# prisma-lab/WBC-quadruped-DOB

Hardware: AMD Instinct MI355X
Metric: WBC control-steps/sec (batched DogBot) (higher is better)
Workload: dtype f64; 1 GPU; configs[1]: batch=4096 states/GPU, 4-contact stance, observer off, f64; synthetic quadruped URDF (DogBot URDF absent); batch_per_gpu=4096, parallelism=batch-sharded x1, no data-path collective, writes_M_h_Jc=True

## Files before the change

### wbc_quadruped_dob_amd/csrc/dyn_split.hip.hpp

```cpp
#pragma once
#include <hip/hip_runtime.h>
#include <type_traits>
#include "device_types.hpp"
#include "dyn_sweep.hip.hpp"

namespace wbc {


#define WBC_LAUNDERED_TID(name) unsigned name = threadIdx.x; asm volatile("" : "+v"(name))
#define WBC_ADDR_MACROS                                                                                                   \
  const size_t N = a.N;                                                                                                    \
  const unsigned N32 = (unsigned)N;                                                                                        \
                                                      \
  const int leg = (int)((tx & 63) >> 4);                                                                          \
     \
  const size_t s_raw = EXT ? (size_t)blockIdx.x * SPW + (tx & 15)                                                 \
                           : ((size_t)blockIdx.x * (BLOCK / 64) + (tx >> 6)) * 16 + (tx & 15);           \
  const bool slot_ok = SPW == 16 || (int)(tx & 15) < SPW;                                                                  \
  const bool live = slot_ok && s_raw < N;                                                                                  \
  unsigned s32 = (unsigned)(live ? s_raw : (slot_ok ? N - 1 : (size_t)blockIdx.x * SPW));                                  \
  const unsigned legN = (unsigned)leg * N32;
#define WBC_STATE_MACROS                                                                                                                          \
  constexpr bool SIMG = EXT == 3;                     \
  const T* const si_ = SIMG ? a.simg + (int)(s32 - (unsigned)((size_t)blockIdx.x * SPW)) : nullptr;                                               \
  auto ldq = [&](int comp) __attribute__((always_inline)) -> T { if constexpr (SIMG) return si_[comp * 16]; else return LDU(a.q, comp); };         \
  auto ldv = [&](int comp) __attribute__((always_inline)) -> T { if constexpr (SIMG) return si_[(SIMG_V + comp) * 16]; else return LDU(a.v, comp); }; \
  (void)ldq; (void)ldv;
#define LDQJ(k_) (SIMG ? si_[(7 + jx[k_]) * 16] : LDX(a.q, 7, jxN[k_]))
#define LDVJ(k_) (SIMG ? si_[(SIMG_V + 6 + jx[k_]) * 16] : LDX(a.v, 6, jxN[k_]))
#define CS(i) cst[(i) * 4 + leg]
#define LDU(ptr, comp) (*(const T*)((const char*)((ptr) + (size_t)(comp) * N) + (size_t)(s32 * (unsigned)sizeof(T))))
#define LDV(ptr, comp) (*(const T*)((const char*)(ptr) + (size_t)(((unsigned)(comp) * N32 + s32) * (unsigned)sizeof(T))))
#define LDX(ptr, c0, xN) (*(const T*)((const char*)((ptr) + (size_t)(c0) * N) + (size_t)(((xN) + s32) * (unsigned)sizeof(T))))
#define WBC_ROLE_LIVE ((0 && EXT != 0) || live)
#define STV(ptr, comp, val) do { if (WBC_ROLE_LIVE) *(T*)((char*)(ptr) + (size_t)(((unsigned)(comp) * N32 + s32) * (unsigned)sizeof(T))) = (val); } while (0)
#define STVG(ptr, comp, val) do { if (live) *(T*)((char*)(ptr) + (size_t)(((unsigned)(comp) * N32 + s32) * (unsigned)sizeof(T))) = (val); } while (0)
#define STL(ptr, c0, stride, val) do { if (WBC_ROLE_LIVE) *(T*)((char*)((ptr) + (size_t)(c0) * N) + (size_t)(((unsigned)(stride) * legN + s32) * (unsigned)sizeof(T))) = (val); } while (0)
#define STLX(ptr, c0, stride, xN, val) do { if (WBC_ROLE_LIVE) *(T*)((char*)((ptr) + (size_t)(c0) * N) + (size_t)(((unsigned)(stride) * legN + (xN) + s32) * (unsigned)sizeof(T))) = (val); } while (0)
#define ST4(ptr, c0, v0_, c1, v1_, c2, v2_, c3, v3_) STV(ptr, sel4<int>(leg, c0, c1, c2, c3), sel4<T>(leg, v0_, v1_, v2_, v3_))
#define ST4G(ptr, c0, v0_, c1, v1_, c2, v2_, c3, v3_) STVG(ptr, sel4<int>(leg, c0, c1, c2, c3), sel4<T>(leg, v0_, v1_, v2_, v3_))
#define MAKE_R(R_, qx, qy, qz, qw) do { const T x = qx, y = qy, z = qz, w = qw; \
    R_.a[0] = 1 - 2 * (y * y + z * z); R_.a[1] = 2 * (x * y - z * w);     R_.a[2] = 2 * (x * z + y * w); \
    R_.a[3] = 2 * (x * y + z * w);     R_.a[4] = 1 - 2 * (x * x + z * z); R_.a[5] = 2 * (y * z - x * w); \
    R_.a[6] = 2 * (x * z - y * w);     R_.a[7] = 2 * (y * z + x * w);     R_.a[8] = 1 - 2 * (x * x + y * y); } while (0)

constexpr int WBC_MJ_WAVES = 2;
constexpr int WBC_RS_WAVES = 2;

template <class T>
WBC_DEV void structural_consts_quarter(const DevModel<T>* __restrict__ model, const SweepArgs<T>& a, const int* zidx_s, unsigned tx) {
  const size_t N = a.N;
  const unsigned N32 = (unsigned)N;
  const int leg = (int)((tx >> 4) & 3), part = (int)(tx >> 6);
  const size_t s_raw = (size_t)blockIdx.x * 16 + (tx & 15);
  const bool live = s_raw < N;
  const unsigned s32 = (unsigned)(live ? s_raw : N - 1);
  const T Z = (T)0;
  int jq[3];
  jidx_of_leg(model, a.jpack, leg, jq);
  const int j0 = jq[0], j1 = jq[1], j2 = jq[2];
  if ((N & 1) == 0) {
    struct alignas(2 * sizeof(T)) T2 { T a, b; };
    const unsigned odd = s32 & 1u, s2 = s32 & ~1u;
#define ST2C(ptr, comp, val) do { if (live) *(T2*)((char*)(ptr) + (size_t)(((unsigned)(comp) * N32 + s2) * (unsigned)sizeof(T))) = T2{(val), (val)}; } while (0)
    if (part == 3) {
      for (int e = 2 * leg + (int)odd; e < 64; e += 8) {
        const int zi = zidx_s[e];
        if (zi >= 0) ST2C(a.M, zi, Z);
      }
    } else {
      const int mrow = part;
      const int rb = 54 * leg + 18 * mrow;
      ST2C(a.Jc, rb + (odd ? 1 : 0), ((odd ? 1 : 0) == mrow) ? (T)1 : Z);
      ST2C(a.Jc, rb + (odd ? 3 + mrow : 2), (!odd && mrow == 2) ? (T)1 : Z);
#pragma unroll
      for (int c = 6; c < 18; c += 2) {
        const int col = c + (int)odd - 6;
        if (col != j0 && col != j1 && col != j2) ST2C(a.Jc, rb + c + (int)odd, Z);
      }
    }
#undef ST2C
  } else {
#define ST1C(ptr, comp, val) do { if (live) *(T*)((char*)(ptr) + (size_t)(((unsigned)(comp) * N32 + s32) * (unsigned)sizeof(T))) = (val); } while (0)
    if (part == 3) {
      for (int e = leg; e < 64; e += 4) {
        const int zi = zidx_s[e];
        if (zi >= 0) ST1C(a.M, zi, Z);
      }
    } else {
      const int mrow = part;
      const int rb = 54 * leg + 18 * mrow;
#pragma unroll
      for (int c = 0; c < 3; ++c) ST1C(a.Jc, rb + c, (c == mrow) ? (T)1 : Z);
      ST1C(a.Jc, rb + 3 + mrow, Z);
#pragma unroll
      for (int c = 0; c < 12; ++c)
        if (c != j0 && c != j1 && c != j2) ST1C(a.Jc, rb + 6 + c, Z);
    }
#undef ST1C
  }
}

constexpr int MJ_HAND_WORDS = 46;
struct MjNoHook { WBC_DEV void operator()() const {} };
template <class T, int BLOCK, int EXT, int SPW = 16, int ZEROS = 1, class AfterHand = MjNoHook>
WBC_DEV void mass_jac_body(const DevModel<T>* __restrict__ model, const SweepArgs<T>& a, const T* cst_ext, const int* zidx_ext, T* hand = nullptr,
                           AfterHand after_hand = AfterHand()) {
  static_assert(!EXT || BLOCK == 64 || BLOCK == 128, "one wavefront (128: one of the two role wavefronts of a fused_pair_kernel workgroup, each with its own half of the parking lot)");
  static_assert(SPW == 16 || EXT != 0, "fewer states per workgroup only for roles");
  WBC_LAUNDERED_TID(tx);
  __shared__ __attribute__((aligned(512))) T cst_own[EXT ? 1 : CST_WORDS];
  __shared__ int zidx_own[EXT ? 1 : 64];
  if constexpr (EXT == 0) {
    for (int i = tx; i < CST_WORDS; i += blockDim.x) cst_own[i] = model->cst[i];
    if (tx < 64) zidx_own[tx] = model->zidx[tx];
    __syncthreads();
  }
  const T* cst = EXT ? cst_ext : cst_own;
  const int* zidx_s = EXT ? zidx_ext : zidx_own;
  WBC_ADDR_MACROS
  WBC_STATE_MACROS
  const bool direct = hand == nullptr;

  T qq[4];
#pragma unroll
  for (int c = 0; c < 4; ++c) qq[c] = ldq(3 + c);
  int jx[3];
  unsigned jxN[3];
  jidx_of_leg(model, a.jpack, leg, jx);
#pragma unroll
  for (int k = 0; k < 3; ++k) jxN[k] = (unsigned)jx[k] * N32;
  T ql[3];
#pragma unroll
  for (int k = 0; k < 3; ++k) ql[k] = LDQJ(k);
  if constexpr (EXT == 2) __syncthreads();

  auto write_consts = [&]() __attribute__((always_inline)) {
    const T Z = (T)0;
    for (int e = leg; e < 64; e += 4) {
      const int zi = zidx_s[e];
      if (zi >= 0) STV(a.M, zi, Z);
    }
#pragma unroll
    for (int mrow = 0; mrow < 3; ++mrow) {
#pragma unroll
      for (int c = 0; c < 3; ++c) STL(a.Jc, 18 * mrow + c, 54, (c == mrow) ? (T)1 : Z);
      STL(a.Jc, 18 * mrow + 3 + mrow, 54, Z);
#pragma unroll
      for (int c = 0; c < 12; ++c)
        if (c != jx[0] && c != jx[1] && c != jx[2]) STL(a.Jc, 18 * mrow + 6 + c, 54, Z);
    }
  };
  if constexpr (ZEROS == 1) { if (!a.skip_consts) write_consts(); }
  T qx, qy, qz, qw;
  {
    const T n = rsqrt_sel<SIMG>(qq[0] * qq[0] + qq[1] * qq[1] + qq[2] * qq[2] + qq[3] * qq[3]);
    qx = qq[0] * n; qy = qq[1] * n; qz = qq[2] * n; qw = qq[3] * n;
  }
  __shared__ T park[18][BLOCK];
  const int ln = EXT ? (int)(tx & (unsigned)(BLOCK - 1)) : (int)tx;
  T* const hl = hand ? hand + (int)(tx & 63) : nullptr;
  M3<T> E2;
#pragma unroll
  for (int k = 0; k < 3; ++k) {
    const int o = JOINT_WORDS * k;
    T sn, cs;
    sincos_t(ql[k], &sn, &cs);
#pragma unroll
    for (int e = 0; e < 9; ++e) {
      const T v = CS(o + e) + cs * CS(o + 9 + e) + sn * CS(o + 18 + e);
      if (k < 2) park[9 * k + e][ln] = v; else E2.a[e] = v;
    }
  }
  T cm; V3<T> ch; S3<T> cI;
  V3<T> dft = mk<T>(CS(129), CS(130), CS(131));
  V3<T> jc[3];
  SF<T> Fp[3];
#pragma unroll
  for (int k = 2; k >= 0; --k) {
    const int o = JOINT_WORDS * k;
    const V3<T> r = mk<T>(CS(o + 27), CS(o + 28), CS(o + 29));
    const V3<T> ax = mk<T>(CS(o + 30), CS(o + 31), CS(o + 32));
    const T m = CS(o + 33);
    const V3<T> h = mk<T>(CS(o + 34), CS(o + 35), CS(o + 36));
    S3<T> Io;
    Io.xx = CS(o + 37); Io.xy = CS(o + 38); Io.xz = CS(o + 39); Io.yy = CS(o + 40); Io.yz = CS(o + 41); Io.zz = CS(o + 42);
    M3<T> E;
    if (k == 2) E = E2;
    else {
#pragma unroll
      for (int e = 0; e < 9; ++e) E.a[e] = park[9 * k + e][ln];
    }
    if (k == 2) { cm = m; ch = h; cI = Io; }
    else {
      cm += m; ch = ch + h;
      cI.xx += Io.xx; cI.xy += Io.xy; cI.xz += Io.xz; cI.yy += Io.yy; cI.yz += Io.yz; cI.zz += Io.zz;
    }
    Fp[k].n = mul(cI, ax);
    Fp[k].f = cross(ax, ch);
#pragma unroll
    for (int j = k; j < 3; ++j) {
      const T mkj = dot(ax, Fp[j].n);
      if (direct) {
        int i = 6 + jx[k], jj = 6 + jx[j];
        if (i > jj) { const int t = i; i = jj; jj = t; }
        STV(a.M, i * 18 - i * (i - 1) / 2 + (jj - i), mkj);
      } else hl[(k * 3 - k * (k - 1) / 2 + (j - k)) * 64] = mkj;
    }
    jc[k] = cross(ax, dft);
    dft = r + mul(E, dft);
#pragma unroll
    for (int j = k; j < 3; ++j) { jc[j] = mul(E, jc[j]); Fp[j] = to_parent(E, r, Fp[j]); }
    {
      const V3<T> hr = mul(E, ch);
      const S3<T> Ir = congr(E, cI);
      const V3<T> w = hr + r * (cm * (T)0.5);
      const T sc = 2 * dot(w, r);
      cI.xx = Ir.xx + sc - 2 * w.x * r.x;
      cI.yy = Ir.yy + sc - 2 * w.y * r.y;
      cI.zz = Ir.zz + sc - 2 * w.z * r.z;
      cI.xy = Ir.xy - (w.x * r.y + r.x * w.y);
      cI.xz = Ir.xz - (w.x * r.z + r.x * w.z);
      cI.yz = Ir.yz - (w.y * r.z + r.y * w.z);
      ch = hr + r * cm;
    }
  }
  M3<T> R;
  MAKE_R(R, qx, qy, qz, qw);
  const V3<T> dw = mul(R, dft);
#pragma unroll
  for (int k = 0; k < 3; ++k) {
    const V3<T> Mf = mul(R, Fp[k].f), Mn = mul(R, Fp[k].n);
    const V3<T> jw = mul(R, jc[k]);
    if (direct) {
      const unsigned x = jxN[k];
      STLX(a.M, 6, 0, x, Mf.x);
      STLX(a.M, midx18(1, 1) + 5, 0, x, Mf.y);
      STLX(a.M, midx18(2, 2) + 4, 0, x, Mf.z);
      STLX(a.M, midx18(3, 3) + 3, 0, x, Mn.x);
      STLX(a.M, midx18(4, 4) + 2, 0, x, Mn.y);
      STLX(a.M, midx18(5, 5) + 1, 0, x, Mn.z);
      STLX(a.Jc, 0 * 18 + 6, 54, x, jw.x);
      STLX(a.Jc, 1 * 18 + 6, 54, x, jw.y);
      STLX(a.Jc, 2 * 18 + 6, 54, x, jw.z);
    } else {
      hl[(6 + 0 + k) * 64] = Mf.x; hl[(6 + 3 + k) * 64] = Mf.y; hl[(6 + 6 + k) * 64] = Mf.z;
      hl[(6 + 9 + k) * 64] = Mn.x; hl[(6 + 12 + k) * 64] = Mn.y; hl[(6 + 15 + k) * 64] = Mn.z;
      hl[(24 + 0 + k) * 64] = jw.x; hl[(24 + 3 + k) * 64] = jw.y; hl[(24 + 6 + k) * 64] = jw.z;
    }
  }
  if (direct) {
    STL(a.Jc, 0 * 18 + 4, 54, dw.z);  STL(a.Jc, 0 * 18 + 5, 54, -dw.y);
    STL(a.Jc, 1 * 18 + 3, 54, -dw.z); STL(a.Jc, 1 * 18 + 5, 54, dw.x);
    STL(a.Jc, 2 * 18 + 3, 54, dw.y);  STL(a.Jc, 2 * 18 + 4, 54, -dw.x);
    if (a.pf) {
      STL(a.pf, 0, 3, ldq(0) + dw.x);
      STL(a.pf, 1, 3, ldq(1) + dw.y);
      STL(a.pf, 2, 3, ldq(2) + dw.z);
    }
  } else {
    hl[33 * 64] = dw.x; hl[34 * 64] = dw.y; hl[35 * 64] = dw.z;
    if (!a.skip_mats && a.pf) {
      STL(a.pf, 0, 3, ldq(0) + dw.x);
      STL(a.pf, 1, 3, ldq(1) + dw.y);
      STL(a.pf, 2, 3, ldq(2) + dw.z);
    }
  }
  {
    const T bm = model->base_m;
    const V3<T> bh = mk<T>(model->base_h[0], model->base_h[1], model->base_h[2]);
    const T tm = xrow_sum(cm) + bm;
    const V3<T> th = xrow_sum(ch) + bh;
    S3<T> tI;
    tI.xx = xrow_sum(cI.xx) + model->base_Io[0]; tI.xy = xrow_sum(cI.xy) + model->base_Io[1]; tI.xz = xrow_sum(cI.xz) + model->base_Io[2];
    tI.yy = xrow_sum(cI.yy) + model->base_Io[3]; tI.yz = xrow_sum(cI.yz) + model->base_Io[4]; tI.zz = xrow_sum(cI.zz) + model->base_Io[5];
    const V3<T> hw = mul(R, th);
    const S3<T> Iw = congr(R, tI);
    if (direct) {
      T* M = a.M;
      ST4(M, midx18(0, 0), tm, midx18(1, 1), tm, midx18(2, 2), tm, midx18(0, 4), hw.z);
      ST4(M, midx18(0, 5), -hw.y, midx18(1, 3), -hw.z, midx18(1, 5), hw.x, midx18(2, 3), hw.y);
      ST4(M, midx18(2, 4), -hw.x, midx18(3, 3), Iw.xx, midx18(3, 4), Iw.xy, midx18(3, 5), Iw.xz);
      if (leg < 3) STV(M, sel4<int>(leg, midx18(4, 4), midx18(4, 5), midx18(5, 5), 0), sel4<T>(leg, Iw.yy, Iw.yz, Iw.zz, Iw.zz));
    } else {
      hl[36 * 64] = tm; hl[37 * 64] = hw.x; hl[38 * 64] = hw.y; hl[39 * 64] = hw.z;
      hl[40 * 64] = Iw.xx; hl[41 * 64] = Iw.xy; hl[42 * 64] = Iw.xz; hl[43 * 64] = Iw.yy; hl[44 * 64] = Iw.yz; hl[45 * 64] = Iw.zz;
    }
  }
  if (!direct) {
    after_hand();
    if (!a.skip_mats) {
#pragma unroll
      for (int k = 0; k < 3; ++k) {
#pragma unroll
        for (int j = k; j < 3; ++j) {
          int i = 6 + jx[k], jj = 6 + jx[j];
          if (i > jj) { const int t = i; i = jj; jj = t; }
          STV(a.M, i * 18 - i * (i - 1) / 2 + (jj - i), hl[(k * 3 - k * (k - 1) / 2 + (j - k)) * 64]);
        }
        const unsigned x = jxN[k];
        STLX(a.M, 6, 0, x, hl[(6 + 0 + k) * 64]);
        STLX(a.M, midx18(1, 1) + 5, 0, x, hl[(6 + 3 + k) * 64]);
        STLX(a.M, midx18(2, 2) + 4, 0, x, hl[(6 + 6 + k) * 64]);
        STLX(a.M, midx18(3, 3) + 3, 0, x, hl[(6 + 9 + k) * 64]);
        STLX(a.M, midx18(4, 4) + 2, 0, x, hl[(6 + 12 + k) * 64]);
        STLX(a.M, midx18(5, 5) + 1, 0, x, hl[(6 + 15 + k) * 64]);
        STLX(a.Jc, 0 * 18 + 6, 54, x, hl[(24 + 0 + k) * 64]);
        STLX(a.Jc, 1 * 18 + 6, 54, x, hl[(24 + 3 + k) * 64]);
        STLX(a.Jc, 2 * 18 + 6, 54, x, hl[(24 + 6 + k) * 64]);
      }
      const T dx = hl[33 * 64], dy = hl[34 * 64], dz = hl[35 * 64];
      STL(a.Jc, 0 * 18 + 4, 54, dz);  STL(a.Jc, 0 * 18 + 5, 54, -dy);
      STL(a.Jc, 1 * 18 + 3, 54, -dz); STL(a.Jc, 1 * 18 + 5, 54, dx);
      STL(a.Jc, 2 * 18 + 3, 54, dy);  STL(a.Jc, 2 * 18 + 4, 54, -dx);
      const T tm = hl[36 * 64], hwx = hl[37 * 64], hwy = hl[38 * 64], hwz = hl[39 * 64];
      T* M = a.M;
      ST4(M, midx18(0, 0), tm, midx18(1, 1), tm, midx18(2, 2), tm, midx18(0, 4), hwz);
      ST4(M, midx18(0, 5), -hwy, midx18(1, 3), -hwz, midx18(1, 5), hwx, midx18(2, 3), hwy);
      ST4(M, midx18(2, 4), -hwx, midx18(3, 3), hl[40 * 64], midx18(3, 4), hl[41 * 64], midx18(3, 5), hl[42 * 64]);
      if (leg < 3) STV(M, sel4<int>(leg, midx18(4, 4), midx18(4, 5), midx18(5, 5), 0), sel4<T>(leg, hl[43 * 64], hl[44 * 64], hl[45 * 64], hl[45 * 64]));
    }
  }
  if constexpr (ZEROS == 2) { if (!a.skip_consts) write_consts(); }
}

template <class T, int BLOCK>
__global__ __launch_bounds__(BLOCK, WBC_MJ_WAVES) void mass_jac_kernel(const DevModel<T>* __restrict__ model, SweepArgs<T> a) {
  mass_jac_body<T, BLOCK, 0>(model, a, nullptr, nullptr);
}

struct NoWait { WBC_DEV void operator()() const {} };
template <class T, int MODE, int BLOCK, int EXT, int SPW = 16, class BeforeRefs = NoWait, class AfterGeom = NoWait, class AfterTaup = NoWait>
WBC_DEV void rnea_step_body(const DevModel<T>* __restrict__ model, const DevParams<T> prm, const SweepArgs<T>& a, const T* cst_ext,
                            T* wsl, BeforeRefs before_refs = BeforeRefs(), AfterGeom after_geom = AfterGeom(), T* hres = nullptr, AfterTaup after_taup = AfterTaup()) {
  static_assert(!EXT || BLOCK == 64 || BLOCK == 128, "one wavefront (128: one of the two role wavefronts of a fused_pair_kernel workgroup, each with its own half of the parking lot)");
  WBC_LAUNDERED_TID(tx);
  constexpr bool WH = (MODE & RS_H) != 0, STEP = (MODE & RS_STEP) != 0, OBS = (MODE & RS_OBS) != 0, WPF = (MODE & RS_PF) != 0, FWD_B = (MODE & RS_NOB) == 0;
  constexpr bool OBSW = (MODE & RS_OBSW) != 0;
  static_assert(!OBSW || (EXT != 0 && OBS && !STEP && !WH), "the observer role exists only inside the fused tick");
  constexpr bool NOJC = (MODE & RS_NOJC) != 0;
  static_assert(!NOJC || (EXT != 0 && STEP && !OBS && !WPF), "RS_NOJC: a step role next to a mass_jac role");
  constexpr bool GEOM = (STEP && !NOJC) || OBS || WPF;
  constexpr bool LANE2 = (MODE & RS_LANE2) != 0;
  static_assert(!LANE2 || (EXT != 0 && SPW == 4 && STEP && WH && !OBS), "RS_LANE2: a role of 4-state workgroups that wants h and tau_partial");
  constexpr bool TWO = STEP && WH && !LANE2;
  constexpr bool BASEROWS = WH || OBS;
  constexpr bool EARLY = EXT != 0 && STEP;
  __shared__ __attribute__((aligned(512))) T cst_own[EXT ? 1 : CST_WORDS];
  if constexpr (EXT == 0) {
    for (int i = tx; i < CST_WORDS; i += blockDim.x) cst_own[i] = model->cst[i];
    __syncthreads();
  }
  const T* cst = EXT ? cst_ext : cst_own;
  WBC_ADDR_MACROS
  const bool chainB = LANE2 && (int)(tx & 15) >= SPW && (int)(tx & 15) < 2 * SPW;
  if constexpr (LANE2) {
    if (chainB) { const size_t sb = (size_t)blockIdx.x * SPW + (tx & 15) - SPW; s32 = (unsigned)(sb < N ? sb : N - 1); }
  }
#define WSTV(comp, val) do { if constexpr (EXT != 0) wsl[(comp) * 16 + (int)(tx & 15)] = (val); else STV(a.ws, comp, val); } while (0)
#define WST4(c0, v0_, c1, v1_, c2, v2_, c3, v3_) WSTV(sel4<int>(leg, c0, c1, c2, c3), sel4<T>(leg, v0_, v1_, v2_, v3_))
#define WSTL(c0, stride, val) WSTV((c0) + (stride) * leg, val)

  WBC_STATE_MACROS
  T qq[4], vb[6];
#pragma unroll
  for (int c = 0; c < 4; ++c) qq[c] = ldq(3 + c);
#pragma unroll
  for (int c = 0; c < 6; ++c) vb[c] = ldv(c);
  T qpos[3] = {0, 0, 0};
  if (WPF && a.pf) {
#pragma unroll
    for (int c = 0; c < 3; ++c) qpos[c] = ldq(c);
  }
  int jx[3];
  unsigned jxN[3];
  jidx_of_leg(model, a.jpack, leg, jx);
#pragma unroll
  for (int k = 0; k < 3; ++k) jxN[k] = (unsigned)jx[k] * N32;
  T ql[3], vl[3], al[3] = {0, 0, 0}, ad[6] = {0, 0, 0, 0, 0, 0};
#pragma unroll
  for (int k = 0; k < 3; ++k) { ql[k] = LDQJ(k); vl[k] = LDVJ(k); }
  constexpr bool LATE_REFS = EARLY && !std::is_same<BeforeRefs, NoWait>::value;
  T bw[6] = {0, 0, 0, 0, 0, 0};
  constexpr bool RIMG = (MODE & RS_REFIMG) != 0;
  static_assert(!RIMG || (SIMG && STEP), "RS_REFIMG: a step role of a 4-state rollout workgroup");
  auto load_refs = [&]() __attribute__((always_inline)) {
    before_refs();
    const T* const ri = RIMG ? a.refimg + (si_ - a.simg) : nullptr;
    if (STEP) {
#pragma unroll
      for (int k = 0; k < 3; ++k) al[k] = RIMG ? ri[(6 + 6 + jx[k]) * 16] : LDX(a.vdot_des, 6, jxN[k]);
#pragma unroll
      for (int c = 0; c < 6; ++c) ad[c] = RIMG ? ri[(6 + c) * 16] : LDU(a.vdot_des, c);
    }
    if (STEP && !OBS && FWD_B) {
#pragma unroll
      for (int c = 0; c < 6; ++c) bw[c] = RIMG ? ri[c * 16] : LDU(a.w_des, c);
    }
  };
  if constexpr (!LATE_REFS) load_refs();
  auto lane2_mask = [&]() __attribute__((always_inline)) {
    if constexpr (LANE2) {
#pragma unroll
      for (int c = 0; c < 6; ++c) { vb[c] = chainB ? (T)0 : vb[c]; ad[c] = chainB ? ad[c] : (T)0; }
#pragma unroll
      for (int k = 0; k < 3; ++k) { vl[k] = chainB ? (T)0 : vl[k]; al[k] = chainB ? al[k] : (T)0; }
    }
  };
  if constexpr (!LATE_REFS) lane2_mask();
  if constexpr (EXT == 2) __syncthreads();
  if constexpr (!EARLY) {
    if (STEP && !OBS && FWD_B) {
      WST4(WS_B + 0, bw[0], WS_B + 1, bw[1], WS_B + 2, bw[2], WS_B + 3, bw[3]);
      if (leg < 2) WSTV(WS_B + 4 + leg, leg == 0 ? bw[4] : bw[5]);
    }
  }
  T qx, qy, qz, qw;
  {
    const T n = rsqrt_sel<(SIMG || (0 && EXT == 2))>(qq[0] * qq[0] + qq[1] * qq[1] + qq[2] * qq[2] + qq[3] * qq[3]);
    qx = qq[0] * n; qy = qq[1] * n; qz = qq[2] * n; qw = qq[3] * n;
  }
  T sn3[3] = {0, 0, 0}, cs3[3] = {0, 0, 0};
  constexpr bool KEEP_E = EARLY && SIMG && SPW == 4;
  M3<T> Ekeep[KEEP_E ? 3 : 1];
  if constexpr (EARLY) {
#pragma unroll
    for (int k = 0; k < 3; ++k) sincos_t(ql[k], &sn3[k], &cs3[k]);
    V3<T> d = mk<T>(CS(129), CS(130), CS(131));
#pragma unroll
    for (int k = 2; k >= 0; --k) {
      const int o = JOINT_WORDS * k;
      T s_ = sn3[k], c_ = cs3[k];
      if constexpr (!KEEP_E) asm volatile("" : "+v"(s_), "+v"(c_));
      M3<T> E;
#pragma unroll
      for (int e = 0; e < 9; ++e) E.a[e] = CS(o + e) + c_ * CS(o + 9 + e) + s_ * CS(o + 18 + e);
      if constexpr (KEEP_E) Ekeep[k] = E;
      d = mk<T>(CS(o + 27), CS(o + 28), CS(o + 29)) + mul(E, d);
    }
    M3<T> R0;
    MAKE_R(R0, qx, qy, qz, qw);
    const V3<T> dw0 = mul(R0, d);
    WSTL(WS_D + 0, 3, dw0.x);
    WSTL(WS_D + 1, 3, dw0.y);
    WSTL(WS_D + 2, 3, dw0.z);
    after_geom();
    if constexpr (LATE_REFS) { load_refs(); lane2_mask(); }
    if (STEP && !OBS && FWD_B) {
      WST4(WS_B + 0, bw[0], WS_B + 1, bw[1], WS_B + 2, bw[2], WS_B + 3, bw[3]);
      if (leg < 2) WSTV(WS_B + 4 + leg, leg == 0 ? bw[4] : bw[5]);
    }
    after_geom();
  }
  const T bm = model->base_m;
  const V3<T> bh = mk<T>(model->base_h[0], model->base_h[1], model->base_h[2]);
  S3<T> bI;
  bI.xx = model->base_Io[0]; bI.xy = model->base_Io[1]; bI.xz = model->base_Io[2];
  bI.yy = model->base_Io[3]; bI.yz = model->base_Io[4]; bI.zz = model->base_Io[5];

  constexpr int PW = 15 + (TWO ? 6 : 0) + (OBS ? 18 : 0);
  constexpr int PB = BASEROWS ? (OBS ? 18 : 6) : 1;
  __shared__ T park[2 * PW + PB][BLOCK];
  const int ln = EXT ? (int)(tx & (unsigned)(BLOCK - 1)) : (int)tx;
  constexpr int OFF_A = 15, OFF_O = 15 + (TWO ? 6 : 0);

  V3<T> omp, vp, aAp, aLp, gLp, a2Ap, a2Lp;
  {
    M3<T> R;
    MAKE_R(R, qx, qy, qz, qw);
    const V3<T> om0 = tmul(R, mk<T>(vb[3], vb[4], vb[5]));
    const V3<T> v0 = tmul(R, mk<T>(vb[0], vb[1], vb[2]));
    V3<T> gneg = tmul(R, mk<T>(-model->grav[0], -model->grav[1], -model->grav[2]));
    if constexpr (LANE2) { gneg.x = chainB ? (T)0 : gneg.x; gneg.y = chainB ? (T)0 : gneg.y; gneg.z = chainB ? (T)0 : gneg.z; }
    const V3<T> aL0 = gneg - cross(om0, v0);
    if (BASEROWS) {
      const SF<T> Iv0 = inertia_mul(bm, bh, bI, om0, v0);
      const SF<T> Ia0 = inertia_mul(bm, bh, bI, mk<T>(0, 0, 0), aL0);
      T* pb = &park[2 * PW][ln];
      const V3<T> bwn = Ia0.n + cross(om0, Iv0.n) + cross(v0, Iv0.f), bwf = Ia0.f + cross(om0, Iv0.f);
      pb[0] = bwn.x; pb[BLOCK] = bwn.y; pb[BLOCK * 2] = bwn.z; pb[BLOCK * 3] = bwf.x; pb[BLOCK * 4] = bwf.y; pb[BLOCK * 5] = bwf.z;
      if (OBS) {
        const V3<T> gn = cross(bh, gneg), gf = gneg * bm;
        pb[BLOCK * 6] = Iv0.n.x; pb[BLOCK * 7] = Iv0.n.y; pb[BLOCK * 8] = Iv0.n.z; pb[BLOCK * 9] = Iv0.f.x; pb[BLOCK * 10] = Iv0.f.y; pb[BLOCK * 11] = Iv0.f.z;
        pb[BLOCK * 12] = gn.x; pb[BLOCK * 13] = gn.y; pb[BLOCK * 14] = gn.z; pb[BLOCK * 15] = gf.x; pb[BLOCK * 16] = gf.y; pb[BLOCK * 17] = gf.z;
      }
    }
    omp = om0; vp = v0; aAp = mk<T>(0, 0, 0); aLp = aL0; gLp = gneg;
    a2Ap = tmul(R, mk<T>(ad[3], ad[4], ad[5]));
    a2Lp = tmul(R, mk<T>(ad[0], ad[1], ad[2]));
    if (STEP && !TWO) { aAp = aAp + a2Ap; aLp = aLp + a2Lp; }
  }

  M3<T> E2;
  SF<T> f2, fa2, m2, g2;
  V3<T> om2, vv2;
#pragma unroll
  for (int k = 0; k < 3; ++k) {
    const int o = JOINT_WORDS * k;
    T sn, cs;
    if constexpr (EARLY) { sn = sn3[k]; cs = cs3[k]; }
    else sincos_t(ql[k], &sn, &cs);
    M3<T> E;
    if constexpr (KEEP_E) E = Ekeep[k];
    else {
#pragma unroll
      for (int e = 0; e < 9; ++e) E.a[e] = CS(o + e) + cs * CS(o + 9 + e) + sn * CS(o + 18 + e);
    }
    const V3<T> r = mk<T>(CS(o + 27), CS(o + 28), CS(o + 29));
    const V3<T> ax = mk<T>(CS(o + 30), CS(o + 31), CS(o + 32));
    const T m = CS(o + 33);
    const V3<T> h = mk<T>(CS(o + 34), CS(o + 35), CS(o + 36));
    S3<T> Io;
    Io.xx = CS(o + 37); Io.xy = CS(o + 38); Io.xz = CS(o + 39); Io.yy = CS(o + 40); Io.yz = CS(o + 41); Io.zz = CS(o + 42);
    const T qd = vl[k];
    const V3<T> om = tmul(E, omp) + ax * qd;
    const V3<T> vv = tmul(E, vp + cross(omp, r));
    V3<T> aA = tmul(E, aAp) + cross(om, ax) * qd;
    const V3<T> aL = tmul(E, aLp + cross(aAp, r)) + cross(vv, ax) * qd;
    if (STEP && !TWO) aA = aA + ax * al[k];
    const SF<T> Iv = inertia_mul(m, h, Io, om, vv);
    const SF<T> Ia = inertia_mul(m, h, Io, aA, aL);
    SF<T> fk, fak, gk;
    fk.n = Ia.n + cross(om, Iv.n) + cross(vv, Iv.f);
    fk.f = Ia.f + cross(om, Iv.f);
    if (TWO) {
      const V3<T> a2A = tmul(E, a2Ap) + ax * al[k];
      const V3<T> a2L = tmul(E, a2Lp + cross(a2Ap, r));
      fak = inertia_mul(m, h, Io, a2A, a2L);
      a2Ap = a2A; a2Lp = a2L;
    }
    if (OBS) {
      const V3<T> gL = tmul(E, gLp);
      gk.n = cross(h, gL);
      gk.f = gL * m;
      gLp = gL;
    }
    if (k < 2) {
      T* pk = &park[PW * k][ln];
#pragma unroll
      for (int e = 0; e < 9; ++e) pk[BLOCK * e] = E.a[e];
      pk[BLOCK * 9] = fk.n.x; pk[BLOCK * 10] = fk.n.y; pk[BLOCK * 11] = fk.n.z;
      pk[BLOCK * 12] = fk.f.x; pk[BLOCK * 13] = fk.f.y; pk[BLOCK * 14] = fk.f.z;
      if (TWO) {
        pk[BLOCK * (OFF_A + 0)] = fak.n.x; pk[BLOCK * (OFF_A + 1)] = fak.n.y; pk[BLOCK * (OFF_A + 2)] = fak.n.z;
        pk[BLOCK * (OFF_A + 3)] = fak.f.x; pk[BLOCK * (OFF_A + 4)] = fak.f.y; pk[BLOCK * (OFF_A + 5)] = fak.f.z;
      }
      if (OBS) {
        pk[BLOCK * (OFF_O + 0)] = Iv.n.x; pk[BLOCK * (OFF_O + 1)] = Iv.n.y; pk[BLOCK * (OFF_O + 2)] = Iv.n.z;
        pk[BLOCK * (OFF_O + 3)] = Iv.f.x; pk[BLOCK * (OFF_O + 4)] = Iv.f.y; pk[BLOCK * (OFF_O + 5)] = Iv.f.z;
        pk[BLOCK * (OFF_O + 6)] = gk.n.x; pk[BLOCK * (OFF_O + 7)] = gk.n.y; pk[BLOCK * (OFF_O + 8)] = gk.n.z;
        pk[BLOCK * (OFF_O + 9)] = gk.f.x; pk[BLOCK * (OFF_O + 10)] = gk.f.y; pk[BLOCK * (OFF_O + 11)] = gk.f.z;
        pk[BLOCK * (OFF_O + 12)] = om.x; pk[BLOCK * (OFF_O + 13)] = om.y; pk[BLOCK * (OFF_O + 14)] = om.z;
        pk[BLOCK * (OFF_O + 15)] = vv.x; pk[BLOCK * (OFF_O + 16)] = vv.y; pk[BLOCK * (OFF_O + 17)] = vv.z;
      }
    } else {
      E2 = E; f2 = fk;
      if (TWO) fa2 = fak;
      if (OBS) { m2 = Iv; g2 = gk; om2 = om; vv2 = vv; }
    }
    omp = om; vp = vv; aAp = aA; aLp = aL;
  }

  T p_leg[3], ct_leg[3], g_leg[3], taup[3] = {0, 0, 0};
  const bool h_mem = !(hres != nullptr && a.skip_mats != 0);
  V3<T> dft = mk<T>(CS(129), CS(130), CS(131));
  V3<T> jc[3];
  SF<T> facc, aacc, macc, gacc;
#pragma unroll
  for (int k = 2; k >= 0; --k) {
    const int o = JOINT_WORDS * k;
    const V3<T> r = mk<T>(CS(o + 27), CS(o + 28), CS(o + 29));
    const V3<T> ax = mk<T>(CS(o + 30), CS(o + 31), CS(o + 32));
    M3<T> E;
    SF<T> fk, fak, mk_, gk;
    V3<T> om, vv;
    if (k == 2) {
      E = E2; fk = f2;
      if (TWO) fak = fa2;
      if (OBS) { mk_ = m2; gk = g2; om = om2; vv = vv2; }
    } else {
      const T* pk = &park[PW * k][ln];
#pragma unroll
      for (int e = 0; e < 9; ++e) E.a[e] = pk[BLOCK * e];
      fk.n = mk<T>(pk[BLOCK * 9], pk[BLOCK * 10], pk[BLOCK * 11]) + facc.n;
      fk.f = mk<T>(pk[BLOCK * 12], pk[BLOCK * 13], pk[BLOCK * 14]) + facc.f;
      if (TWO) {
        fak.n = mk<T>(pk[BLOCK * (OFF_A + 0)], pk[BLOCK * (OFF_A + 1)], pk[BLOCK * (OFF_A + 2)]) + aacc.n;
        fak.f = mk<T>(pk[BLOCK * (OFF_A + 3)], pk[BLOCK * (OFF_A + 4)], pk[BLOCK * (OFF_A + 5)]) + aacc.f;
      }
      if (OBS) {
        mk_.n = mk<T>(pk[BLOCK * (OFF_O + 0)], pk[BLOCK * (OFF_O + 1)], pk[BLOCK * (OFF_O + 2)]) + macc.n;
        mk_.f = mk<T>(pk[BLOCK * (OFF_O + 3)], pk[BLOCK * (OFF_O + 4)], pk[BLOCK * (OFF_O + 5)]) + macc.f;
        gk.n = mk<T>(pk[BLOCK * (OFF_O + 6)], pk[BLOCK * (OFF_O + 7)], pk[BLOCK * (OFF_O + 8)]) + gacc.n;
        gk.f = mk<T>(pk[BLOCK * (OFF_O + 9)], pk[BLOCK * (OFF_O + 10)], pk[BLOCK * (OFF_O + 11)]) + gacc.f;
        om = mk<T>(pk[BLOCK * (OFF_O + 12)], pk[BLOCK * (OFF_O + 13)], pk[BLOCK * (OFF_O + 14)]);
        vv = mk<T>(pk[BLOCK * (OFF_O + 15)], pk[BLOCK * (OFF_O + 16)], pk[BLOCK * (OFF_O + 17)]);
      }
    }
    {
      const T hk = dot(ax, fk.n);
      if (WH) {
        unsigned long long jp = a.jpack;
        asm volatile("" : "+s"(jp));
        const unsigned jx_k = ((unsigned)(jp >> (12 * leg)) >> (4 * k)) & 15u;
        const unsigned jxN_k = jx_k * N32;
        if (h_mem) STLX(a.h, 6, 0, jxN_k, hk);
        if (hres) hres[(6 + (int)jx_k) * 16 + (int)(tx & 15)] = hk;
      }
      if (STEP) taup[k] = hk + (TWO ? dot(ax, fak.n) : (T)0);
    }
    if (OBS) {
      p_leg[k] = dot(ax, mk_.n);
      ct_leg[k] = -dot(ax, cross(om, mk_.n) + cross(vv, mk_.f));
      g_leg[k] = dot(ax, gk.n);
    }
    if (GEOM) {
      jc[k] = cross(ax, dft);
      dft = r + mul(E, dft);
#pragma unroll
      for (int j = k; j < 3; ++j) jc[j] = mul(E, jc[j]);
    }
    if (k > 0 || BASEROWS) facc = to_parent(E, r, fk);
    if (TWO && k > 0) aacc = to_parent(E, r, fak);
    if (OBS) { macc = to_parent(E, r, mk_); gacc = to_parent(E, r, gk); }
  }

  M3<T> R;
  MAKE_R(R, qx, qy, qz, qw);
  V3<T> dw = mk<T>(0, 0, 0), jw[3];
  if (GEOM) {
    dw = mul(R, dft);
#pragma unroll
    for (int k = 0; k < 3; ++k) jw[k] = mul(R, jc[k]);
  }
  if (WPF && a.pf) {
    STL(a.pf, 0, 3, qpos[0] + dw.x);
    STL(a.pf, 1, 3, qpos[1] + dw.y);
    STL(a.pf, 2, 3, qpos[2] + dw.z);
  }
  if (STEP) {
    if constexpr (!EARLY) {
      WSTL(WS_D + 0, 3, dw.x);
      WSTL(WS_D + 1, 3, dw.y);
      WSTL(WS_D + 2, 3, dw.z);
    }
    if constexpr (GEOM) {
#pragma unroll
      for (int k = 0; k < 3; ++k) {
        WSTL(WS_JCL + 0 + k, 9, jw[k].x);
        WSTL(WS_JCL + 3 + k, 9, jw[k].y);
        WSTL(WS_JCL + 6 + k, 9, jw[k].z);
      }
    }
  }
  constexpr bool TAUP_FIRST = STEP && !OBS && !OBSW && WH && !std::is_same<AfterTaup, NoWait>::value;
  if constexpr (TAUP_FIRST) {
    if constexpr (LANE2) {
#pragma unroll
      for (int k = 0; k < 3; ++k) taup[k] += dpp_mov<0x12C>(taup[k]);
    }
#pragma unroll
    for (int k = 0; k < 3; ++k) WSTL(WS_TAUP + k, 3, taup[k]);
    after_taup();
  }
  if (WH) {
    const T* pb = &park[2 * PW][ln];
    const V3<T> bfn = xrow_sum(facc.n) + mk<T>(pb[0], pb[BLOCK], pb[BLOCK * 2]);
    const V3<T> bff = xrow_sum(facc.f) + mk<T>(pb[BLOCK * 3], pb[BLOCK * 4], pb[BLOCK * 5]);
    const V3<T> hb_f = mul(R, bff), hb_n = mul(R, bfn);
    if (h_mem) {
      ST4(a.h, 0, hb_f.x, 1, hb_f.y, 2, hb_f.z, 3, hb_n.x);
      if (leg < 2) STV(a.h, 4 + leg, leg == 0 ? hb_n.y : hb_n.z);
    }
    if (hres) {
      hres[sel4<int>(leg, 0, 1, 2, 3) * 16 + (int)(tx & 15)] = sel4<T>(leg, hb_f.x, hb_f.y, hb_f.z, hb_n.x);
      if (leg < 2) hres[(4 + leg) * 16 + (int)(tx & 15)] = leg == 0 ? hb_n.y : hb_n.z;
    }
  }
  T p_b[6], beta_b[6], beta_l[3];
  if (OBS) {
    const T* pb = &park[2 * PW][ln];
    SF<T> mom0, grv0;
    mom0.n = xrow_sum(macc.n) + mk<T>(pb[BLOCK * 6], pb[BLOCK * 7], pb[BLOCK * 8]);
    mom0.f = xrow_sum(macc.f) + mk<T>(pb[BLOCK * 9], pb[BLOCK * 10], pb[BLOCK * 11]);
    grv0.n = xrow_sum(gacc.n) + mk<T>(pb[BLOCK * 12], pb[BLOCK * 13], pb[BLOCK * 14]);
    grv0.f = xrow_sum(gacc.f) + mk<T>(pb[BLOCK * 15], pb[BLOCK * 16], pb[BLOCK * 17]);
    const V3<T> Pl = mul(R, mom0.f), Pa = mul(R, mom0.n);
    const V3<T> gl = mul(R, grv0.f), ga = mul(R, grv0.n);
    const V3<T> cx = cross(mk<T>(vb[0], vb[1], vb[2]), Pl);
    p_b[0] = Pl.x; p_b[1] = Pl.y; p_b[2] = Pl.z; p_b[3] = Pa.x; p_b[4] = Pa.y; p_b[5] = Pa.z;
    beta_b[0] = -gl.x; beta_b[1] = -gl.y; beta_b[2] = -gl.z;
    beta_b[3] = -cx.x - ga.x; beta_b[4] = -cx.y - ga.y; beta_b[5] = -cx.z - ga.z;
#pragma unroll
    for (int k = 0; k < 3; ++k) beta_l[k] = ct_leg[k] - g_leg[k];
    if (a.p) {
      ST4(a.p, 0, p_b[0], 1, p_b[1], 2, p_b[2], 3, p_b[3]);
      if (leg < 2) STV(a.p, 4 + leg, leg == 0 ? p_b[4] : p_b[5]);
#pragma unroll
      for (int k = 0; k < 3; ++k) STLX(a.p, 6, 0, jxN[k], p_leg[k]);
    }
    if (a.beta) {
      ST4(a.beta, 0, beta_b[0], 1, beta_b[1], 2, beta_b[2], 3, beta_b[3]);
      if (leg < 2) STV(a.beta, 4 + leg, leg == 0 ? beta_b[4] : beta_b[5]);
#pragma unroll
      for (int k = 0; k < 3; ++k) STLX(a.beta, 6, 0, jxN[k], beta_l[k]);
    }
  }
  if (STEP || OBSW) {
    T rb[6] = {0, 0, 0, 0, 0, 0}, rl[3] = {0, 0, 0};
    if (OBS && prm.observer_order > 0) {
      const V3<T> fp = mk<T>(LDV(a.f_prev, 3 * leg + 0), LDV(a.f_prev, 3 * leg + 1), LDV(a.f_prev, 3 * leg + 2));
      const V3<T> ub_f = xrow_sum(fp);
      const V3<T> ub_n = xrow_sum(cross(dw, fp));
      const T ub[6] = {ub_f.x, ub_f.y, ub_f.z, ub_n.x, ub_n.y, ub_n.z};
      const T dt = prm.dt;
      const bool o1 = prm.observer_order == 1;
#pragma unroll
      for (int c = 0; c < 6; ++c) {
        const T r0 = LDU(a.obs_r, c);
        const T ig = LDU(a.obs_integ, c) + dt * (ub[c] + beta_b[c] + r0);
        const T e = p_b[c] - ig;
        rb[c] = o1 ? prm.K1[c] * e : r0 + dt * prm.K2[c] * (prm.K1[c] * e - r0);
        p_b[c] = ig;
      }
      ST4G(a.obs_integ, 0, p_b[0], 1, p_b[1], 2, p_b[2], 3, p_b[3]);
      if (leg < 2) STVG(a.obs_integ, 4 + leg, leg == 0 ? p_b[4] : p_b[5]);
      ST4G(a.obs_r, 0, rb[0], 1, rb[1], 2, rb[2], 3, rb[3]);
      if (leg < 2) STVG(a.obs_r, 4 + leg, leg == 0 ? rb[4] : rb[5]);
#pragma unroll
      for (int k = 0; k < 3; ++k) {
        const int c = 6 + jx[k];
        const T r0 = LDV(a.obs_r, c);
        const T u = LDV(a.tau_prev, jx[k]) + dot(jw[k], fp);
        const T ig = LDV(a.obs_integ, c) + dt * (u + beta_l[k] + r0);
        const T e = p_leg[k] - ig;
        T k1 = prm.K1[6], k2 = prm.K2[6];
#pragma unroll
        for (int j = 1; j < 12; ++j) { k1 = (jx[k] == j) ? prm.K1[6 + j] : k1; k2 = (jx[k] == j) ? prm.K2[6 + j] : k2; }
        rl[k] = o1 ? k1 * e : r0 + dt * k2 * (k1 * e - r0);
        STVG(a.obs_integ, c, ig);
        STVG(a.obs_r, c, rl[k]);
      }
    }
    if constexpr (OBSW) {
      WST4(WS_RHAT + 0, rb[0], WS_RHAT + 1, rb[1], WS_RHAT + 2, rb[2], WS_RHAT + 3, rb[3]);
      if (leg < 2) WSTV(WS_RHAT + 4 + leg, leg == 0 ? rb[4] : rb[5]);
#pragma unroll
      for (int k = 0; k < 3; ++k) WSTL(WS_RHAT + 6 + k, 3, rl[k]);
    } else {
      if (OBS) {
        T b[6];
#pragma unroll
        for (int c = 0; c < 6; ++c) b[c] = LDU(a.w_des, c) - rb[c];
        WST4(WS_B + 0, b[0], WS_B + 1, b[1], WS_B + 2, b[2], WS_B + 3, b[3]);
        if (leg < 2) WSTV(WS_B + 4 + leg, leg == 0 ? b[4] : b[5]);
      }
      if constexpr (!TAUP_FIRST) {
      if constexpr (LANE2) {
#pragma unroll
        for (int k = 0; k < 3; ++k) taup[k] += dpp_mov<0x12C>(taup[k]);
      }
#pragma unroll
      for (int k = 0; k < 3; ++k) WSTL(WS_TAUP + k, 3, taup[k] - rl[k]);
      }
    }
  }
#undef WSTL
#undef WST4
#undef WSTV
}

template <class T, int MODE, int BLOCK>
__global__ __launch_bounds__(BLOCK, WBC_RS_WAVES) void rnea_step_kernel(const DevModel<T>* __restrict__ model, DevParams<T> prm,
                                                                         SweepArgs<T> a) {
  if (a.qp_todo && blockIdx.x == 0 && threadIdx.x == 0) a.qp_todo[0] = 0;
  rnea_step_body<T, MODE, BLOCK, 0>(model, prm, a, nullptr, nullptr);
}

#undef MAKE_R
#undef ST4
#undef ST4G
#undef STVG
#undef STLX
#undef STL
#undef STV
#undef LDX
#undef LDV
#undef LDU
#undef CS

}
```

### wbc_quadruped_dob_amd/csrc/fused_tick.hip.hpp

```cpp
#pragma once
#include <hip/hip_runtime.h>
#include "device_types.hpp"
#include "dyn_split.hip.hpp"
#include "qp_struct16.hip.hpp"
#include "integrate.hip.hpp"
#include "com_ref.hip.hpp"
#include "observer.hip.hpp"

namespace wbc {

constexpr int FUSED_OBS_WAVES = 2;

template <class T, bool OBSERVER, bool MATS, bool WARM = false> constexpr bool fused_split_h() {
  return !OBSERVER && MATS && WARM && sizeof(T) == 8;
}
template <class T, bool OBSERVER, bool MATS, bool WARM = false> constexpr int fused_threads() { return OBSERVER ? 384 + 64 * FUSED_OBS_WAVES : (fused_split_h<T, OBSERVER, MATS, WARM>() ? 448 : 384); }
template <class T, bool OBSERVER, bool MATS, bool WARM = false>
__global__ __launch_bounds__((fused_threads<T, OBSERVER, MATS, WARM>()), 1) void fused_tick_kernel(const DevModel<T>* __restrict__ model, DevParams<T> prm,
                                                                            SweepArgs<T> a, QpArgs<T> qa, QpJidx jmap) {
  __shared__ __attribute__((aligned(512))) T cst[CST_WORDS];
  __shared__ int zidx_s[64];
  __shared__ T wsl[WS_LDS_WORDS * 16];
  __shared__ int ready, gready, oready;
  __shared__ int rpack;
  constexpr bool SPEC_ORDER = OBSERVER && !WARM;
  const int wave = (int)(threadIdx.x >> 6);
#ifdef WBC_FUSED_STAMP
  double* const stamp = (double*)a.pf;
  const unsigned stampN = (unsigned)a.N;
  a.pf = nullptr;
#define FSTAMP(slot) do { if (stamp) WBC_FSTAMP(stamp, stampN, slot); } while (0)
  if (wave == 0) FSTAMP(0);
#else
#define FSTAMP(slot) do {} while (0)
#endif
  if (wave == 4) {
    int* const gflag = &gready;
    constexpr int RMODE = (MATS && !fused_split_h<T, OBSERVER, MATS, WARM>()) ? (RS_STEP | RS_H) : RS_STEP;
    auto geom_out = [=] __device__() {
      __builtin_amdgcn_fence(__ATOMIC_RELEASE, "workgroup", "local");
      if ((threadIdx.x & 63) == 0) __hip_atomic_fetch_add(gflag, 1, __ATOMIC_RELAXED, __HIP_MEMORY_SCOPE_WORKGROUP);
      FSTAMP(7);
    };
    rnea_step_body<T, RMODE, 64, 2>(model, prm, a, cst, wsl, NoWait(), geom_out);
    FSTAMP(8);
    __builtin_amdgcn_fence(__ATOMIC_RELEASE, "workgroup", "local");
    if ((threadIdx.x & 63) == 0) __hip_atomic_fetch_add(&ready, 1, __ATOMIC_RELAXED, __HIP_MEMORY_SCOPE_WORKGROUP);
  } else if (wave == 5) {
    if constexpr (MATS) mass_jac_body<T, 64, 2, 16, (0)>(model, a, cst, zidx_s);
    else __syncthreads();
    FSTAMP(9);
  } else if (fused_split_h<T, OBSERVER, MATS, WARM>() && wave == 6) {
    if constexpr (fused_split_h<T, OBSERVER, MATS, WARM>()) rnea_step_body<T, RS_H, 64, 2>(model, prm, a, cst, wsl);
  } else if (OBSERVER && wave == 6) {
    if constexpr (OBSERVER) {
      int* const ack = &rpack;
      auto wait_ack = [ack] __device__() {
        if constexpr (SPEC_ORDER) { while (__hip_atomic_load(ack, __ATOMIC_RELAXED, __HIP_MEMORY_SCOPE_WORKGROUP) < 4) __builtin_amdgcn_s_sleep(1); }
      };
      observer_body<T, 64, 2, 1, 16, decltype(wait_ack)>(model, prm, a, cst, wsl, wait_ack);
      __builtin_amdgcn_fence(__ATOMIC_RELEASE, "workgroup", "local");
      if ((threadIdx.x & 63) == 0) __hip_atomic_fetch_add(&oready, 1, __ATOMIC_RELAXED, __HIP_MEMORY_SCOPE_WORKGROUP);
      FSTAMP(10);
    }
  } else if (OBSERVER && FUSED_OBS_WAVES == 2 && wave == 7) {
    if constexpr (OBSERVER && FUSED_OBS_WAVES == 2) {
      observer_body<T, 64, 2, 2>(model, prm, a, cst, wsl);
      __builtin_amdgcn_fence(__ATOMIC_RELEASE, "workgroup", "local");
      if ((threadIdx.x & 63) == 0) __hip_atomic_fetch_add(&ready, 1, __ATOMIC_RELAXED, __HIP_MEMORY_SCOPE_WORKGROUP);
    }
  } else {
    for (int i = threadIdx.x; i < CST_WORDS; i += 256) cst[i] = model->cst[i];
    if (threadIdx.x < 64) zidx_s[threadIdx.x] = model->zidx[threadIdx.x];
    if (threadIdx.x == 0) { ready = 0; gready = 0; oready = 0; rpack = 0; }
    __syncthreads();
    constexpr int NFIN = (OBSERVER && FUSED_OBS_WAVES == 2) ? 2 : 1;
#ifdef WBC_FUSED_STAMP
    QpSync sy{&gready, &oready, &ready, 1, 2, 1, NFIN, stamp, stampN};
#else
    QpSync sy{&gready, &oready, &ready, 1, 2, 1, NFIN};
#endif
    if constexpr (SPEC_ORDER) sy.rp_ack = &rpack;
    if constexpr (MATS) {
      const int* const zs = zidx_s;
      const unsigned tq = threadIdx.x;
      auto idle = [=] __device__() { if (!a.skip_consts) structural_consts_quarter<T>(model, a, zs, tq); };
      qp_body<T, true, OBSERVER, 16, false, 4, decltype(idle), false, WARM ? 1 : 0>(prm, qa, jmap, wsl, &sy, QpWho{0, false}, idle);
    } else
    qp_body<T, true, OBSERVER, 16, false, 4, QpNoIdle, false, WARM ? 1 : 0>(prm, qa, jmap, wsl, &sy);
  }
}

template <class P> WBC_DEV void shift_ptr(P*& p, int off) { if (p) p += off; }
template <class T> WBC_DEV void shift_states(SweepArgs<T>& a, int off) {
  shift_ptr(a.q, off); shift_ptr(a.v, off); shift_ptr(a.M, off); shift_ptr(a.h, off); shift_ptr(a.Jc, off); shift_ptr(a.pf, off); shift_ptr(a.p, off); shift_ptr(a.beta, off);
  shift_ptr(a.w_des, off); shift_ptr(a.vdot_des, off); shift_ptr(a.tau_prev, off); shift_ptr(a.f_prev, off); shift_ptr(a.obs_integ, off); shift_ptr(a.obs_r, off); shift_ptr(a.ws, off);
}
template <class T> WBC_DEV void shift_states(QpArgs<T>& a, int off) {
  shift_ptr(a.ws, off); shift_ptr(a.normals, off); shift_ptr(a.mu, off); shift_ptr(a.mask, off); shift_ptr(a.Jc, off); shift_ptr(a.wdes, off);
  shift_ptr(a.tau, off); shift_ptr(a.f, off); shift_ptr(a.status, off); shift_ptr(a.iters, off); shift_ptr(a.aset_in, off); shift_ptr(a.aset_out, off); shift_ptr(a.rprev, off);
}
constexpr int FUSED_PAIR_THREADS = 768;
template <class T>
__global__ __launch_bounds__(FUSED_PAIR_THREADS) void fused_pair_kernel(const DevModel<T>* __restrict__ model, DevParams<T> prm, SweepArgs<T> a, QpArgs<T> qa, QpJidx jmap) {
  __shared__ __attribute__((aligned(512))) T cst[CST_WORDS];
  __shared__ int zidx_s[64];
  __shared__ T wsl2[2 * WS_LDS_WORDS * 16];
  __shared__ int flags[2][4];
  const int wave = (int)(threadIdx.x >> 6);
  const int half = __builtin_amdgcn_readfirstlane(wave < 8 ? (wave >> 2) : (wave & 1));
  const int pairs = (int)(a.N >> 5);
  const bool tail = (int)blockIdx.x == pairs;
  const int off = tail ? (int)a.N - 32 + 16 * half - 16 * pairs : (half ? 16 * pairs : 0);
  T* const wsl = wsl2 + half * (WS_LDS_WORDS * 16);
  int* const ready = &flags[half][0];
  int* const gready = &flags[half][1];
  int* const oready = &flags[half][2];
  if (wave >= 8) {
    shift_states(a, off);
    if (wave < 10) {
      auto geom_out = [=] __device__() {
        __builtin_amdgcn_fence(__ATOMIC_RELEASE, "workgroup", "local");
        if ((threadIdx.x & 63) == 0) __hip_atomic_fetch_add(gready, 1, __ATOMIC_RELAXED, __HIP_MEMORY_SCOPE_WORKGROUP);
      };
      rnea_step_body<T, RS_STEP | RS_H, 128, 2>(model, prm, a, cst, wsl, NoWait(), geom_out);
      __builtin_amdgcn_fence(__ATOMIC_RELEASE, "workgroup", "local");
      if ((threadIdx.x & 63) == 0) __hip_atomic_fetch_add(ready, 1, __ATOMIC_RELAXED, __HIP_MEMORY_SCOPE_WORKGROUP);
    } else {
      mass_jac_body<T, 128, 2, 16, (0)>(model, a, cst, zidx_s);
    }
  } else {
    for (int i = threadIdx.x; i < CST_WORDS; i += 512) cst[i] = model->cst[i];
    if (threadIdx.x < 64) zidx_s[threadIdx.x] = model->zidx[threadIdx.x];
    if (threadIdx.x < 8) (&flags[0][0])[threadIdx.x] = 0;
    __syncthreads();
    shift_states(a, off);
    shift_states(qa, half ? off - 16 : off);
#ifdef WBC_FUSED_STAMP
    QpSync sy{gready, oready, ready, 1, 2, 1, 1, nullptr, 0};
#else
    QpSync sy{gready, oready, ready, 1, 2, 1, 1};
#endif
    const int* const zs = zidx_s;
    const unsigned tq = threadIdx.x & 255u;
    auto idle = [=] __device__() { if (!a.skip_consts) structural_consts_quarter<T>(model, a, zs, tq); };
    qp_body<T, true, false, 16, false, 8, decltype(idle), false, 0>(prm, qa, jmap, wsl - (half ? 16 : 0), &sy, QpWho{0, false}, idle);
  }
}

__host__ __device__ constexpr int rollout_threads(bool observer, int spw) {
  return (spw == 4) ? (256)
       : (spw == 16) ? (observer ? 512 : 384)
       : (observer ? 512 : 448);
}
template <class T, bool OBSERVER, bool TRACK, int SPW = 16, bool WARM = false, bool PAYLOAD = false>
__global__ __launch_bounds__(rollout_threads(OBSERVER, SPW), 1) void rollout_kernel(const DevModel<T>* __restrict__ model, DevParams<T> prm,
                                                                         SweepArgs<T> a, QpArgs<T> qa, QpJidx jmap, IntegrateArgsP<T, PAYLOAD> ia,
                                                                         int horizon, const DevRefParams<T>* __restrict__ G, RefArgs<T> ra) {
#define WBC_RB_SCORE 0
#include "rollout_body.inc.hpp"
#undef WBC_RB_SCORE
}
template <class T, bool OBSERVER, bool TRACK, int SPW = 16, bool PAYLOAD = false>
__global__ __launch_bounds__(rollout_threads(OBSERVER, SPW), 1) void rollout_scored_kernel(const DevModel<T>* __restrict__ model, DevParams<T> prm,
                                                                         SweepArgs<T> a, QpArgs<T> qa, QpJidx jmap, IntegrateArgsP<T, PAYLOAD> ia,
                                                                         int horizon, const DevRefParams<T>* __restrict__ G, RefArgs<T> ra, ScoreArgs<T> sc) {
  constexpr bool WARM = true;
  const ScoreArgs<T>* const sca = &sc;
#define WBC_RB_SCORE 1
#include "rollout_body.inc.hpp"
#undef WBC_RB_SCORE
}

}
```

Baseline: 307.7 million control-steps/s.

## Enable split-h wave for cold f64 ticks and move structural constants onto it

Measured after the change: 305.9 million control-steps/s. Within noise of the previous version (-0.6%).

```diff
diff --git a/wbc_quadruped_dob_amd/csrc/dyn_split.hip.hpp b/wbc_quadruped_dob_amd/csrc/dyn_split.hip.hpp
--- a/wbc_quadruped_dob_amd/csrc/dyn_split.hip.hpp
+++ b/wbc_quadruped_dob_amd/csrc/dyn_split.hip.hpp
@@ -330,9 +330,10 @@
 }
 
 struct NoWait { WBC_DEV void operator()() const {} };
-template <class T, int MODE, int BLOCK, int EXT, int SPW = 16, class BeforeRefs = NoWait, class AfterGeom = NoWait, class AfterTaup = NoWait>
+template <class T, int MODE, int BLOCK, int EXT, int SPW = 16, class BeforeRefs = NoWait, class AfterGeom = NoWait, class AfterTaup = NoWait, class AfterTables = NoWait>
 WBC_DEV void rnea_step_body(const DevModel<T>* __restrict__ model, const DevParams<T> prm, const SweepArgs<T>& a, const T* cst_ext,
-                            T* wsl, BeforeRefs before_refs = BeforeRefs(), AfterGeom after_geom = AfterGeom(), T* hres = nullptr, AfterTaup after_taup = AfterTaup()) {
+                            T* wsl, BeforeRefs before_refs = BeforeRefs(), AfterGeom after_geom = AfterGeom(), T* hres = nullptr, AfterTaup after_taup = AfterTaup(),
+                            AfterTables after_tables = AfterTables()) {
   static_assert(!EXT || BLOCK == 64 || BLOCK == 128, "one wavefront (128: one of the two role wavefronts of a fused_pair_kernel workgroup, each with its own half of the parking lot)");
   WBC_LAUNDERED_TID(tx);
   constexpr bool WH = (MODE & RS_H) != 0, STEP = (MODE & RS_STEP) != 0, OBS = (MODE & RS_OBS) != 0, WPF = (MODE & RS_PF) != 0, FWD_B = (MODE & RS_NOB) == 0;
@@ -408,7 +409,7 @@
     }
   };
   if constexpr (!LATE_REFS) lane2_mask();
-  if constexpr (EXT == 2) __syncthreads();
+  if constexpr (EXT == 2) { __syncthreads(); after_tables(); }
   if constexpr (!EARLY) {
     if (STEP && !OBS && FWD_B) {
       WST4(WS_B + 0, bw[0], WS_B + 1, bw[1], WS_B + 2, bw[2], WS_B + 3, bw[3]);
diff --git a/wbc_quadruped_dob_amd/csrc/fused_tick.hip.hpp b/wbc_quadruped_dob_amd/csrc/fused_tick.hip.hpp
--- a/wbc_quadruped_dob_amd/csrc/fused_tick.hip.hpp
+++ b/wbc_quadruped_dob_amd/csrc/fused_tick.hip.hpp
@@ -7,12 +7,19 @@
 #include "com_ref.hip.hpp"
 #include "observer.hip.hpp"
 
+#ifndef WBC_COLD_CONSTS_LAST
+#define WBC_COLD_CONSTS_LAST 0
+#endif
+
 namespace wbc {
 
 constexpr int FUSED_OBS_WAVES = 2;
 
 template <class T, bool OBSERVER, bool MATS, bool WARM = false> constexpr bool fused_split_h() {
-  return !OBSERVER && MATS && WARM && sizeof(T) == 8;
+  return !OBSERVER && MATS && sizeof(T) == 8;
+}
+template <class T, bool OBSERVER, bool MATS, bool WARM = false> constexpr bool fused_consts_on_h() {
+  return fused_split_h<T, OBSERVER, MATS, WARM>() && !WARM;
 }
 template <class T, bool OBSERVER, bool MATS, bool WARM = false> constexpr int fused_threads() { return OBSERVER ? 384 + 64 * FUSED_OBS_WAVES : (fused_split_h<T, OBSERVER, MATS, WARM>() ? 448 : 384); }
 template <class T, bool OBSERVER, bool MATS, bool WARM = false>
@@ -30,9 +37,11 @@
   const unsigned stampN = (unsigned)a.N;
   a.pf = nullptr;
 #define FSTAMP(slot) do { if (stamp) WBC_FSTAMP(stamp, stampN, slot); } while (0)
+#define FSTAMP_C(slot, col) do { if (stamp && (threadIdx.x & 63) == 0) stamp[(size_t)(slot) * stampN + (size_t)blockIdx.x * 16 + (col)] = (double)wall_clock64(); } while (0)
   if (wave == 0) FSTAMP(0);
 #else
 #define FSTAMP(slot) do {} while (0)
+#define FSTAMP_C(slot, col) do {} while (0)
 #endif
   if (wave == 4) {
     int* const gflag = &gready;
@@ -51,7 +60,28 @@
     else __syncthreads();
     FSTAMP(9);
   } else if (fused_split_h<T, OBSERVER, MATS, WARM>() && wave == 6) {
-    if constexpr (fused_split_h<T, OBSERVER, MATS, WARM>()) rnea_step_body<T, RS_H, 64, 2>(model, prm, a, cst, wsl);
+    if constexpr (fused_consts_on_h<T, OBSERVER, MATS, WARM>()) {
+      const int* const zs = zidx_s;
+      const unsigned lane = threadIdx.x & 63u;
+      auto consts = [=] __device__() {
+        if (!a.skip_consts) {
+#pragma unroll 1
+          for (unsigned part = 0; part < 4; ++part) structural_consts_quarter<T>(model, a, zs, lane + 64u * part);
+        }
+        FSTAMP_C(1, 1);
+      };
+#if WBC_COLD_CONSTS_LAST
+      rnea_step_body<T, RS_H, 64, 2>(model, prm, a, cst, wsl);
+      FSTAMP_C(0, 1);
+      consts();
+#else
+      rnea_step_body<T, RS_H, 64, 2>(model, prm, a, cst, wsl, NoWait(), NoWait(), nullptr, NoWait(), consts);
+      FSTAMP_C(0, 1);
+#endif
+    } else if constexpr (fused_split_h<T, OBSERVER, MATS, WARM>()) {
+      rnea_step_body<T, RS_H, 64, 2>(model, prm, a, cst, wsl);
+      FSTAMP_C(0, 1);
+    }
   } else if (OBSERVER && wave == 6) {
     if constexpr (OBSERVER) {
       int* const ack = &rpack;
@@ -81,7 +111,7 @@
     QpSync sy{&gready, &oready, &ready, 1, 2, 1, NFIN};
 #endif
     if constexpr (SPEC_ORDER) sy.rp_ack = &rpack;
-    if constexpr (MATS) {
+    if constexpr (MATS && !fused_consts_on_h<T, OBSERVER, MATS, WARM>()) {
       const int* const zs = zidx_s;
       const unsigned tq = threadIdx.x;
       auto idle = [=] __device__() { if (!a.skip_consts) structural_consts_quarter<T>(model, a, zs, tq); };
```
